# kishwarshafin/pepper

Hardware: AMD Instinct MI355X
Metric: inference windows/sec (whole node) (higher is better)
Workload: dtype f32 via f16 hi/lo split operands (3 MFMAs per product), f32 accumulate

## Files before the change

### pepper_amd/csrc/rnn_h2.hip

```cpp
#include <cstdlib>

#include "common.h"
#include "kernels.h"

namespace {

typedef _Float16 h8 __attribute__((ext_vector_type(8)));
typedef float f32x2 __attribute__((ext_vector_type(2)));

constexpr int MT = 64;

PA_DEV f32x16 mfma_h(h8 a, h8 b, f32x16 c) { return __builtin_amdgcn_mfma_f32_32x32x16_f16(a, b, c, 0, 0, 0); }

PA_DEV void decode_block(int bid, int& dir, int& btile) {
    const int xcd = bid & 7, q = bid >> 3;
    dir = xcd >> 2;
    btile = q * 4 + (xcd & 3);
}


extern __shared__ __attribute__((aligned(16))) uint32_t lds[];
template <int MTILES, int KXROW = 0, int XRD_ = 0>
struct LstmLds {
    static_assert(MTILES == 1 || MTILES == 2, "32 or 64 rows per workgroup");
    static constexpr int H = 256, NW = H / 32;
    static constexpr int MTL = 32 * MTILES;
    static constexpr int ROWB = (H + KXROW) * 4 + 16;
    static constexpr int ROWD = ROWB / 4;
    static_assert((ROWB / 16) % 2 == 1, "row stride must be an odd number of 16-byte slots");
    static constexpr int CS = NW * MTILES * 16 * 64;
    static constexpr int XRD = XRD_, XSLOT = MTL * XRD;
    static constexpr int RING = MTL * ROWD + CS;
    static constexpr size_t BYTES = (size_t)(RING + 2 * XSLOT) * 4;
    static_assert(BYTES <= 160 * 1024, "a workgroup has one CU's 160 KB of LDS");
    PA_DEV static float* c_slots(int u, int lane) { return reinterpret_cast<float*>(lds + MTL * ROWD) + u * (MTILES * 16 * 64) + lane; }
    PA_DEV static void clear(int tid) {
        for (int idx = tid; idx < RING; idx += blockDim.x) lds[idx] = 0u;
    }
};

template <int MTILES> using SeedLds = LstmLds<MTILES>;
template <int MTILES> using EncLds = LstmLds<MTILES, 32>;
template <int MTILES> using DecLds = LstmLds<MTILES, 0, 36>;

PA_DEV f32x2 lstm_gate_pair(f32x2 ai, f32x2 af, f32x2 ag, f32x2 ao, float* c) {
    const f32x2 one = {1.0f, 1.0f};
    auto ex2 = [](f32x2 v) { return f32x2{__builtin_amdgcn_exp2f(v.x), __builtin_amdgcn_exp2f(v.y)}; };
    auto rcp = [](f32x2 v) { return f32x2{__builtin_amdgcn_rcpf(v.x), __builtin_amdgcn_rcpf(v.y)}; };
    const f32x2 ig = rcp(one + ex2(ai));
    const f32x2 fg = rcp(one + ex2(af));
    const f32x2 gg = one - 2.0f * rcp(one + ex2(ag));
    const f32x2 og = rcp(one + ex2(ao));
    const f32x2 cold = {c[0], c[64]};
    const f32x2 cn = fg * cold + ig * gg;
    c[0] = cn.x;
    c[64] = cn.y;
    return og * (one - 2.0f * rcp(one + ex2(cn * 2.8853900817779268f)));
}

template <int ROWD, int MTL, int AUX>
struct YCopy {
    static constexpr int CPR = 256 / 4;
    static constexpr int YROWS = 512 / CPR;
    static constexpr int YC = MTL / YROWS;
    const uint32_t* src;
    __amdgpu_buffer_rsrc_t rs;
    unsigned off;
    int T, ldy;
    PA_DEV YCopy(uint32_t* Y, int ldy_, int b0, int T_, int dir, int tid) : T(T_), ldy(ldy_) {
        const int row = tid / CPR, c = tid % CPR;
        src = lds + row * ROWD + c * 4;
        rs = __builtin_amdgcn_make_buffer_rsrc(Y + (size_t)b0 * T * ldy + dir * 256, 0, 0x7fffffff, 0x00020000);
        off = ((unsigned)(row * T) * ldy + c * 4) * 4u;
    }
    PA_DEV u32x4 read(int j) const { return *reinterpret_cast<const u32x4*>(src + j * YROWS * ROWD); }
    PA_DEV void write(int j, int tp, u32x4 v) const {
        __builtin_amdgcn_raw_buffer_store_b128(v, rs, off, ((unsigned)(j * YROWS * T + tp) * ldy) * 4u, AUX);
    }
};

template <int MTILES>
__global__ __launch_bounds__(512, 1) void lstm_seed_h2_kernel(const float* __restrict__ Xp, int ldx, const uint32_t* __restrict__ Wp,
                                                              uint32_t* __restrict__ Y, int ldy, int B, int T,
                                                              unsigned long long* __restrict__ dbg) {
    using L = SeedLds<MTILES>;
    constexpr int H = 256, KS = H / 16, NT = H / 32;
    constexpr int MTL = L::MTL, ROWD = L::ROWD;
    static_assert(KS % 2 == 0, "the weight prefetch assumes an even number of k steps");

    int dir, btile;
    decode_block(blockIdx.x, dir, btile);
    const int b0 = btile * MTL;
    if (b0 >= B) return;

    const int tid = threadIdx.x, lane = tid & 63;
    const int u = __builtin_amdgcn_readfirstlane(tid >> 6);
    const int li = lane & 31, hf = lane >> 5;
    float* cs = L::c_slots(u, lane);
    L::clear(tid);

    f32x16 acc[MTILES][4];

    const __amdgpu_buffer_rsrc_t xrs = __builtin_amdgcn_make_buffer_rsrc(
        const_cast<float*>(Xp + (size_t)(b0 >> 5) * T * (ldx >> 5) * 1024), 0, 0x7fffffff, 0x00020000);
    const __amdgpu_buffer_rsrc_t wrs = __builtin_amdgcn_make_buffer_rsrc(
        const_cast<uint32_t*>(Wp + ((size_t)dir * (4 * NT) + u) * KS * 512), 0, 0x7fffffff, 0x00020000);
    const unsigned xoff = lane * 16u;
    const unsigned woff = lane * 16u;

    auto seed_chunk = [&](int m, int qd, int t) {
#pragma unroll
        for (int g = 0; g < 4; ++g) {
            const unsigned ct = (unsigned)(dir * (4 * NT) + g * NT + u);
            const unsigned so = (((unsigned)(m * T + t) * (ldx >> 5) + ct) * 4u + qd) * 1024u;
            const f32x4 v = __builtin_bit_cast(f32x4, __builtin_amdgcn_raw_buffer_load_b128(xrs, xoff, so, 0));
            acc[m][g][4 * qd] = v.x;
            acc[m][g][4 * qd + 1] = v.y;
            acc[m][g][4 * qd + 2] = v.z;
            acc[m][g][4 * qd + 3] = v.w;
        }
    };

    struct Frag { h8 b[4][2], a[MTILES][2]; };
    const uint32_t* arow = lds + li * ROWD + hf * 8;
    auto load_b = [&](int s, Frag& fr) {
#pragma unroll
        for (int g = 0; g < 4; ++g)
#pragma unroll
            for (int hl = 0; hl < 2; ++hl)
                fr.b[g][hl] = __builtin_bit_cast(h8, __builtin_amdgcn_raw_buffer_load_b128(
                                                         wrs, woff, (unsigned)((g * NT * KS + s) * 2 + hl) * 1024u, 0));
    };
    auto load_a = [&](int s, Frag& fr) {
#pragma unroll
        for (int m = 0; m < MTILES; ++m) {
            fr.a[m][0] = *reinterpret_cast<const h8*>(arow + m * 32 * ROWD + s * 16);
            fr.a[m][1] = *reinterpret_cast<const h8*>(arow + m * 32 * ROWD + s * 16 + 4);
        }
    };

    const YCopy<ROWD, MTL, 0> yc(Y, ldy, b0, T, dir, tid);
    constexpr int YC = decltype(yc)::YC;

    const int hcol = 32 * u + li;
    unsigned short* hl_dst = reinterpret_cast<unsigned short*>(lds + 4 * hf * ROWD + (hcol >> 3) * 8 + ((hcol & 7) >> 1)) + (hcol & 1);

    Frag ring[2];
    __syncthreads();
    {
        const int t0 = dir ? T - 1 : 0;
#pragma unroll
        for (int m = 0; m < MTILES; ++m)
#pragma unroll
            for (int qd = 0; qd < 4; ++qd) seed_chunk(m, qd, t0);
        load_b(0, ring[0]);
    }
    __syncthreads();

    for (int step = 0; step < T; ++step) {
        const int t = dir ? T - 1 - step : step;
        const bool stamp = dbg != nullptr && blockIdx.x == 8 && lane == 0;
        if (stamp) dbg[(u * 80 + 2 * step) * 2] = __builtin_amdgcn_s_memtime();
        {
            load_a(0, ring[0]);
            const int tp = step > 0 ? (dir ? t + 1 : t - 1) : t;
            u32x4 ycv = {0, 0, 0, 0};
#pragma unroll
            for (int s = 0; s < KS; ++s) {
                const int p = s & 1;
                if (s + 1 < KS) { load_b(s + 1, ring[p ^ 1]); load_a(s + 1, ring[p ^ 1]); }
                else load_b(0, ring[p ^ 1]);
                if (s >= 1 && s <= YC) yc.write(s - 1, tp, ycv);
                if (s < YC) ycv = yc.read(s);
#pragma unroll
                for (int term = 0; term < 3; ++term)
#pragma unroll
                    for (int g = 0; g < 4; ++g)
#pragma unroll
                        for (int m = 0; m < MTILES; ++m)
                            acc[m][g] = mfma_h(ring[p].a[m][term == 0 ? 1 : 0], ring[p].b[g][term == 1 ? 1 : 0], acc[m][g]);
                if (MTILES == 1 && s + 1 < KS) {
#pragma unroll
                    for (int q = 0; q < 8; ++q) {
                        __builtin_amdgcn_sched_group_barrier(0x008, 1, 0);
                        __builtin_amdgcn_sched_group_barrier(0x020, 1, 0);
                    }
#pragma unroll
                    for (int q = 0; q < 2; ++q) {
                        __builtin_amdgcn_sched_group_barrier(0x008, 1, 0);
                        __builtin_amdgcn_sched_group_barrier(0x100, 1, 0);
                    }
                    if (s <= YC) {
                        __builtin_amdgcn_sched_group_barrier(0x008, 1, 0);
                        __builtin_amdgcn_sched_group_barrier(0x040, 1, 0);
                        __builtin_amdgcn_sched_group_barrier(0x008, 1, 0);
                        __builtin_amdgcn_sched_group_barrier(0x100, 1, 0);
                    } else {
                        __builtin_amdgcn_sched_group_barrier(0x008, 2, 0);
                    }
                } else if (s + 1 < KS) {
#pragma unroll
                    for (int q = 0; q < 8; ++q) {
                        __builtin_amdgcn_sched_group_barrier(0x008, 2, 0);
                        __builtin_amdgcn_sched_group_barrier(0x020, 1, 0);
                    }
#pragma unroll
                    for (int q = 0; q < 4; ++q) {
                        __builtin_amdgcn_sched_group_barrier(0x008, 1, 0);
                        __builtin_amdgcn_sched_group_barrier(0x100, 1, 0);
                    }
                    if (s <= YC) {
                        __builtin_amdgcn_sched_group_barrier(0x008, 1, 0);
                        __builtin_amdgcn_sched_group_barrier(0x040, 1, 0);
                        __builtin_amdgcn_sched_group_barrier(0x008, 1, 0);
                        __builtin_amdgcn_sched_group_barrier(0x100, 1, 0);
                        __builtin_amdgcn_sched_group_barrier(0x008, 2, 0);
                    } else {
                        __builtin_amdgcn_sched_group_barrier(0x008, 4, 0);
                    }
                } else if (MTILES == 1) {
#pragma unroll
                    for (int q = 0; q < 8; ++q) {
                        __builtin_amdgcn_sched_group_barrier(0x008, 1, 0);
                        __builtin_amdgcn_sched_group_barrier(0x020, 1, 0);
                    }
                    __builtin_amdgcn_sched_group_barrier(0x008, 4, 0);
                } else {
#pragma unroll
                    for (int q = 0; q < 8; ++q) {
                        __builtin_amdgcn_sched_group_barrier(0x008, 2, 0);
                        __builtin_amdgcn_sched_group_barrier(0x020, 1, 0);
                    }
                    __builtin_amdgcn_sched_group_barrier(0x008, 8, 0);
                }
                __builtin_amdgcn_sched_barrier(0);
            }
        }
        if (stamp) dbg[(u * 80 + 2 * step) * 2 + 1] = __builtin_amdgcn_s_memtime();

        lds_barrier();
        if (stamp) dbg[(u * 80 + 2 * step + 1) * 2] = __builtin_amdgcn_s_memtime();

        const int tn = dir ? t - 1 : t + 1;
#pragma unroll
        for (int m = 0; m < MTILES; ++m)
#pragma unroll
            for (int qd = 0; qd < 4; ++qd) {
#pragma unroll
                for (int e = 0; e < 4; e += 2) {
                    const int r = 4 * qd + e;
                    const f32x2 ai = {acc[m][0][r], acc[m][0][r + 1]}, af = {acc[m][1][r], acc[m][1][r + 1]},
                                ag = {acc[m][2][r], acc[m][2][r + 1]}, ao = {acc[m][3][r], acc[m][3][r + 1]};
                    const f32x2 hv2 = lstm_gate_pair(ai, af, ag, ao, cs + (m * 16 + r) * 64);
#pragma unroll
                    for (int k = 0; k < 2; ++k)
                        h2_store16(hl_dst + (32 * m + ((r + k) & 3) + 8 * ((r + k) >> 2)) * ROWD * 2, k ? hv2.y : hv2.x);
                }
                if (step + 1 < T) seed_chunk(m, qd, tn);
            }
        if (stamp) dbg[(u * 80 + 2 * step + 1) * 2 + 1] = __builtin_amdgcn_s_memtime();
        lds_barrier();
    }
    {
        const int tl = dir ? 0 : T - 1;
#pragma unroll
        for (int j = 0; j < YC; ++j) yc.write(j, tl, yc.read(j));
    }
}


template <int KS>
PA_DEV __amdgpu_buffer_rsrc_t frag16_rsrc(const uint32_t* Wp, int dir, int u) {
    return __builtin_amdgcn_make_buffer_rsrc(const_cast<uint32_t*>(Wp + ((size_t)dir * (4 * 16) + 2 * u) * KS * 512), 0, 0x7fffffff,
                                             0x00020000);
}
template <int KS>
PA_DEV void load_b16(h8 (&b)[2][2][2][2], __amdgpu_buffer_rsrc_t wrs, unsigned woff, int s, int gp, int idx) {
    const int c = idx >> 2, hl = (idx >> 1) & 1, g2 = idx & 1;
    b[gp][g2][c][hl] = __builtin_bit_cast(
        h8, __builtin_amdgcn_raw_buffer_load_b128(wrs, woff, (unsigned)((((2 * gp + g2) * 16 + c) * KS + s) * 2 + hl) * 1024u, 0));
}
PA_DEV __amdgpu_buffer_rsrc_t bias16_rsrc(const float* bias, int dir, int u) {
    return __builtin_amdgcn_make_buffer_rsrc(const_cast<float*>(bias + dir * 4 * 256 + 32 * u), 0, 0x7fffffff, 0x00020000);
}
PA_DEV void load_bias16(float (&cb)[4][2], __amdgpu_buffer_rsrc_t brs, int lr) {
#pragma unroll
    for (int g = 0; g < 4; ++g)
#pragma unroll
        for (int c = 0; c < 2; ++c)
            cb[g][c] = __builtin_bit_cast(float, __builtin_amdgcn_raw_buffer_load_b32(brs, lr * 4u, (unsigned)(g * 256 + 16 * c) * 4u, 0));
}
template <int ROWD>
PA_DEV unsigned short* hl_dst16(int hcol, int lq) {
    return reinterpret_cast<unsigned short*>(lds + 4 * lq * ROWD + (hcol >> 3) * 8 + ((hcol & 7) >> 1)) + (hcol & 1);
}
template <int ROWD, bool ADD_BIAS>
PA_DEV void gate_tile16(f32x4 i4, f32x4 f4, f32x4 g4, f32x4 o4, f32x4 b4, float* cs, unsigned short* dst) {
#pragma unroll
    for (int e = 0; e < 4; e += 2) {
        f32x2 ai = {i4[e], i4[e + 1]}, af = {f4[e], f4[e + 1]}, ag = {g4[e], g4[e + 1]}, ao = {o4[e], o4[e + 1]};
        if (ADD_BIAS) { ai += b4[0]; af += b4[1]; ag += b4[2]; ao += b4[3]; }
        const f32x2 hv2 = lstm_gate_pair(ai, af, ag, ao, cs + e * 64);
#pragma unroll
        for (int k = 0; k < 2; ++k) h2_store16(dst + (e + k) * ROWD * 2, k ? hv2.y : hv2.x);
    }
}

template <bool FRESH_, bool Y_, bool Y2_, int XR_, int AN_>
struct DecStep {
    static constexpr bool FRESH = FRESH_, Y = Y_, Y2 = Y2_;
    static constexpr int XR = XR_, AN = AN_;
};

template <int MTILES>
PA_DEV void lstm_dec_h2_body(const uint32_t* __restrict__ Xh, int ldxh, const float* __restrict__ bias,
                             const uint32_t* __restrict__ Wp, uint32_t* __restrict__ Y, int ldy, int B, int T,
                             unsigned long long* __restrict__ dbg) {
    using L = DecLds<MTILES>;
    constexpr int H = 256, KX = 512, KS = (H + KX) / 32, KSH = H / 32, SAUX = 2;
    constexpr int MTL = L::MTL, RT = 2 * MTILES, ROWD = L::ROWD, XRD = L::XRD, XSLOT = L::XSLOT;

    int dir, btile;
    decode_block(blockIdx.x, dir, btile);
    const int b0 = btile * MTL;
    if (b0 >= B) return;

    const int tid = threadIdx.x, lane = tid & 63;
    const int u = __builtin_amdgcn_readfirstlane(tid >> 6);
    const int lr = lane & 15, lq = lane >> 4;
    float* cs = L::c_slots(u, lane);
    L::clear(tid);
    uint32_t* xring = lds + L::RING;

    f32x4 acc[RT][4][2];

    const __amdgpu_buffer_rsrc_t brs = bias16_rsrc(bias, dir, u);
    const __amdgpu_buffer_rsrc_t wrs = frag16_rsrc<KS>(Wp, dir, u);
    const unsigned woff = lane * 16u;

    const bool xg_stager = tid < MTL * 8;
    const __amdgpu_buffer_rsrc_t xgrs =
        __builtin_amdgcn_make_buffer_rsrc(const_cast<uint32_t*>(Xh + (size_t)b0 * T * ldxh), 0, 0x7fffffff, 0x00020000);
    const unsigned xg_off = ((unsigned)((tid >> 3) * T) * ldxh) * 4u + (tid & 7) * 16u;
    uint32_t* xst_dst = xring + (tid >> 3) * XRD + (tid & 7) * 4;
    u32x4 xstage = {0, 0, 0, 0};
    auto xg_load = [&](int j, int t) {
        if (MTILES == 2 || xg_stager)
            xstage = __builtin_amdgcn_raw_buffer_load_b128(xgrs, xg_off, ((unsigned)t * ldxh) * 4u + (unsigned)j * 128u, SAUX);
    };
    auto xg_store = [&](int slot) {
        if (MTILES == 2 || xg_stager) *reinterpret_cast<u32x4*>(xst_dst + slot * XSLOT) = xstage;
    };

    int once = 1;
    asm volatile("" : "+s"(once));
    h8 a[RT][2];
    h8 b[2][2][2][2];
    const uint32_t* arow = lds + lr * ROWD + lq * 8;
    const uint32_t* xrow = xring + lr * XRD + lq * 8;
    auto load_b = [&](int s, int gp, int idx) { load_b16<KS>(b, wrs, woff, s, gp, idx); };
    auto load_a_h = [&](int s, int m, int hl) { a[m][hl] = *reinterpret_cast<const h8*>(arow + m * 16 * ROWD + s * 32 + hl * 4); };
    auto load_a_x = [&](int slot, int m, int hl) {
        a[m][hl] = *reinterpret_cast<const h8*>(xrow + slot * XSLOT + m * 16 * XRD + hl * 4);
    };

    const YCopy<ROWD, MTL, SAUX> yc(Y, ldy, b0, T, dir, tid);
    constexpr int YC = decltype(yc)::YC;
    unsigned short* hl_dst = hl_dst16<ROWD>(32 * u + lr, lq);

    __syncthreads();
#pragma unroll
    for (int i = 0; i < 8; ++i) load_b(0, 0, i);
    __syncthreads();

    for (int step = 0; step < T; ++step) {
        const int t = dir ? T - 1 - step : step;
        const bool stamp = dbg != nullptr && blockIdx.x == 8 && lane == 0;
        if (stamp) dbg[(u * 80 + 2 * step) * 2] = __builtin_amdgcn_s_memtime();
        {
            const int tp = step > 0 ? (dir ? t + 1 : t - 1) : t;
            u32x4 ycv = {0, 0, 0, 0}, ycv2 = {0, 0, 0, 0};
            constexpr int NM = RT * 12;
            auto kstep = [&](int s, auto cfg) {
                using C = decltype(cfg);
                const int sn = C::AN == 0 ? 0 : s + 1, slot = (s - KSH + 1) & 1;
#pragma unroll
                for (int gp = 0; gp < 2; ++gp) {
                    if (gp == 1 && C::XR == 2) lds_barrier();
#pragma unroll
                    for (int i = 0; i < NM; ++i) {
                        const int m = i / 12, c = (i % 12) / 6, term = (i % 6) >> 1, g2 = i & 1, g = 2 * gp + g2;
                        acc[m][g][c] = __builtin_amdgcn_mfma_f32_16x16x32_f16(a[m][term == 0 ? 1 : 0], b[gp][g2][c][term == 1 ? 1 : 0],
                                                                              C::FRESH && term == 0 ? f32x4{} : acc[m][g][c], 0, 0, 0);
                        if (MTILES == 2 ? (i < 24 && i % 3 == 1) : i < 8) load_b(gp == 0 ? s : sn, gp ^ 1, MTILES == 2 ? i / 3 : i);
                        if (gp == 1 && C::AN != 0 && (i % 12 == 9 || i % 12 == 11)) {
                            if (C::AN == 1) load_a_h(sn, m, i % 12 == 9 ? 1 : 0);
                            else load_a_x(slot, m, i % 12 == 9 ? 1 : 0);
                        }
                        if (C::Y && i == NM / 2 + 1) {
                            if (gp == 0) ycv = yc.read(s);
                            else yc.write(s, tp, ycv);
                        }
                        if (C::Y2 && i == NM / 2 + 4) {
                            if (gp == 0) ycv2 = yc.read(YC - 1);
                            else yc.write(YC - 1, tp, ycv2);
                        }
                        if (C::XR == 2 && gp == 0 && i == NM - 1) xg_store(slot);
                        if (C::XR != 0 && gp == 1 && i == (MTILES == 2 ? 2 : 10)) xg_load(s - 6 < KS - KSH ? s - 6 : KS - KSH - 1, t);
                        __builtin_amdgcn_sched_barrier(0);
                    }
                }
            };
            constexpr bool Y2 = YC > 7;
            constexpr int YL = YC < 6 ? YC : 6;
#pragma unroll
            for (int i = 0; i < 2 * RT; ++i) load_a_h(0, i >> 1, i & 1);
            __builtin_amdgcn_sched_barrier(0);
#pragma unroll 1
            for (int r = 0; r < once; ++r) kstep(0, DecStep<true, true, Y2, 0, 1>{});
#pragma unroll 1
            for (int s = 1; s < YL; ++s) kstep(s, DecStep<false, true, false, 0, 1>{});
#pragma unroll 1
            for (int s = YL; s < 6; ++s) kstep(s, DecStep<false, false, false, 0, 1>{});
#pragma unroll 1
            for (int r = 0; r < once; ++r) kstep(6, DecStep<false, (YC > 6), false, 1, 1>{});
#pragma unroll 1
            for (int s = 7; s < KS - 1; ++s) kstep(s, DecStep<false, false, false, 2, 2>{});
#pragma unroll 1
            for (int r = 0; r < once; ++r) kstep(KS - 1, DecStep<false, false, false, 0, 0>{});
        }
        float cb[4][2];
        load_bias16(cb, brs, lr);
        if (stamp) dbg[(u * 80 + 2 * step) * 2 + 1] = __builtin_amdgcn_s_memtime();

        lds_barrier();
        if (stamp) dbg[(u * 80 + 2 * step + 1) * 2] = __builtin_amdgcn_s_memtime();

#pragma unroll
        for (int m = 0; m < RT; ++m)
#pragma unroll
            for (int c = 0; c < 2; ++c)
                gate_tile16<ROWD, true>(acc[m][0][c], acc[m][1][c], acc[m][2][c], acc[m][3][c], f32x4{cb[0][c], cb[1][c], cb[2][c], cb[3][c]},
                                        cs + (m * 8 + c * 4) * 64, hl_dst + 16 * m * ROWD * 2 + c * 32);
        if (stamp) dbg[(u * 80 + 2 * step + 1) * 2 + 1] = __builtin_amdgcn_s_memtime();
        lds_barrier();
    }
    {
        const int tl = dir ? 0 : T - 1;
#pragma unroll
        for (int j = 0; j < YC; ++j) yc.write(j, tl, yc.read(j));
    }
}

template <bool FRESH_, bool Y_, bool X_, int AN_>
struct EncStep {
    static constexpr bool FRESH = FRESH_, Y = Y_, X = X_;
    static constexpr int AN = AN_;
};

template <int MTILES, bool BC>
PA_DEV void lstm_enc_h2_body(const int8_t* __restrict__ Xi, int F, const float* __restrict__ bias, const uint32_t* __restrict__ Wp,
                             uint32_t* __restrict__ Y, int ldy, int B, int T, unsigned long long* __restrict__ dbg) {
    constexpr int H = 256, KX = 32, KS = (H + KX) / 32, KSH = H / 32, NW = H / 32, SAUX = 2;
    using L = EncLds<MTILES>;
    constexpr int MTL = L::MTL, RT = 2 * MTILES, ROWD = L::ROWD;

    int dir, btile;
    decode_block(blockIdx.x, dir, btile);
    const int b0 = btile * MTL;
    if (b0 >= B) return;

    const int tid = threadIdx.x, lane = tid & 63;
    const int u = __builtin_amdgcn_readfirstlane(tid >> 6);
    const int lr = lane & 15, lq = lane >> 4;
    float* cs = L::c_slots(u, lane);
    L::clear(tid);

    f32x4 acc[RT][4][2];

    const __amdgpu_buffer_rsrc_t brs = bias16_rsrc(bias, dir, u);
    const __amdgpu_buffer_rsrc_t wrs = frag16_rsrc<KS>(Wp, dir, u);
    const unsigned woff = lane * 16u;

    constexpr int XN = (MTL * KX / 2) / (NW * 64);
    unsigned xv[XN];
    auto x_load = [&](int t) {
#pragma unroll
        for (int k = 0; k < XN; ++k) {
            const int e = tid + k * (NW * 64);
            const int row = e / (KX / 2), f = (e % (KX / 2)) * 2;
            int brow = b0 + row;
            brow = brow < B ? brow : B - 1;
            const int8_t* src = Xi + ((size_t)brow * T + t) * F;
            const _Float16 one = BC ? (_Float16)1.0f : (_Float16)0.0f;
            const _Float16 h0 = f < F ? (_Float16)(float)src[f] : (f == F ? one : (_Float16)0.0f);
            const _Float16 h1 = f + 1 < F ? (_Float16)(float)src[f + 1] : (f + 1 == F ? one : (_Float16)0.0f);
            xv[k] = (unsigned)__builtin_bit_cast(unsigned short, h0) | ((unsigned)__builtin_bit_cast(unsigned short, h1) << 16);
        }
    };
    auto x_store = [&]() {
#pragma unroll
        for (int k = 0; k < XN; ++k) {
            const int e = tid + k * (NW * 64);
            const int row = e / (KX / 2), f = (e % (KX / 2)) * 2;
            lds[row * ROWD + ((H + f) >> 3) * 8 + ((f & 7) >> 1)] = xv[k];
        }
    };

    int once = 1;
    asm volatile("" : "+s"(once));
    h8 a[RT][2];
    h8 b[2][2][2][2];
    const uint32_t* arow = lds + lr * ROWD + lq * 8;
    auto load_b = [&](int s, int gp, int idx) { load_b16<KS>(b, wrs, woff, s, gp, idx); };
    auto load_a = [&](int s, int m, int hl) { a[m][hl] = *reinterpret_cast<const h8*>(arow + m * 16 * ROWD + s * 32 + hl * 4); };

    const YCopy<ROWD, MTL, SAUX> yc(Y, ldy, b0, T, dir, tid);
    constexpr int YC = decltype(yc)::YC;
    static_assert(YC <= KSH, "one y copy pass per h k step");
    unsigned short* hl_dst = hl_dst16<ROWD>(32 * u + lr, lq);

    __syncthreads();
    {
        x_load(dir ? T - 1 : 0);
        x_store();
#pragma unroll
        for (int i = 0; i < 8; ++i) load_b(KS - 1, 0, i);
    }
    __syncthreads();

    for (int step = 0; step < T; ++step) {
        const int t = dir ? T - 1 - step : step;
        const bool stamp = dbg != nullptr && blockIdx.x == 8 && lane == 0;
        if (stamp) dbg[(u * 80 + 2 * step) * 2] = __builtin_amdgcn_s_memtime();
        {
            const int tp = step > 0 ? (dir ? t + 1 : t - 1) : t;
            u32x4 ycv = {0, 0, 0, 0};
            auto kstep = [&](int s, auto cfg) {
                using C = decltype(cfg);
                constexpr int PT = C::X ? 4 : 6;
                constexpr int NM = RT * 2 * PT;
                const int sn = C::X ? 0 : s + 1;
#pragma unroll
                for (int gp = 0; gp < 2; ++gp) {
#pragma unroll
                    for (int i = 0; i < NM; ++i) {
                        const int m = i / (2 * PT), c = (i % (2 * PT)) / PT, term = ((i % PT) >> 1) + (C::X ? 1 : 0), g2 = i & 1,
                                  g = 2 * gp + g2;
                        acc[m][g][c] = __builtin_amdgcn_mfma_f32_16x16x32_f16(a[m][term == 0 ? 1 : 0], b[gp][g2][c][term == 1 ? 1 : 0],
                                                                              C::FRESH && i % PT < 2 ? f32x4{} : acc[m][g][c], 0, 0, 0);
                        if (C::X) {
                            if (MTILES == 2 ? (i < 16 && (i & 1)) : i < 8) load_b(gp == 0 ? s : sn, gp ^ 1, MTILES == 2 ? i >> 1 : i);
                        } else {
                            if (MTILES == 2 ? (i < 24 && i % 3 == 1) : i < 8) load_b(gp == 0 ? s : sn, gp ^ 1, MTILES == 2 ? i / 3 : i);
                        }
                        if (!C::X && gp == 1 && C::AN == 1 && i % 12 == 9) load_a(sn, m, 1);
                        if (!C::X && gp == 1 && C::AN != 0 && i % 12 == 11) load_a(sn, m, 0);
                        if (C::Y && i == NM / 2 + 1) {
                            if (gp == 0) ycv = yc.read(s);
                            else yc.write(s, tp, ycv);
                        }
                        __builtin_amdgcn_sched_barrier(0);
                    }
                }
            };
            const int hrun = step == 0 ? 0 : once;
#pragma unroll
            for (int i = 0; i < 2 * RT; ++i) load_a(0, i >> 1, i & 1);
            __builtin_amdgcn_sched_barrier(0);
#pragma unroll 1
            for (int r = 0; r < hrun; ++r) kstep(0, EncStep<true, true, false, 1>{});
#pragma unroll 1
            for (int s = 1; s < (YC < KSH - 1 ? YC : KSH - 1) * hrun; ++s) kstep(s, EncStep<false, true, false, 1>{});
            if constexpr (YC < KSH - 1) {
#pragma unroll 1
                for (int s = YC; s < (KSH - 1) * hrun; ++s) kstep(s, EncStep<false, false, false, 1>{});
            }
#pragma unroll 1
            for (int r = 0; r < hrun; ++r) kstep(KSH - 1, EncStep<false, (YC >= KSH), false, 2>{});
#pragma unroll 1
            for (int r = 0; r < hrun; ++r) kstep(KS - 1, EncStep<false, false, true, 0>{});
#pragma unroll 1
            for (int r = hrun; r < once; ++r) {
#pragma unroll
                for (int m = 0; m < RT; ++m) load_a(KSH, m, 0);
                __builtin_amdgcn_sched_barrier(0);
                kstep(KS - 1, EncStep<true, false, true, 0>{});
            }
        }
        float cb[4][2] = {};
        if (!BC) load_bias16(cb, brs, lr);
        if (stamp) dbg[(u * 80 + 2 * step) * 2 + 1] = __builtin_amdgcn_s_memtime();

        lds_barrier();
        if (stamp) dbg[(u * 80 + 2 * step + 1) * 2] = __builtin_amdgcn_s_memtime();

        const int tn = dir ? t - 1 : t + 1;
        if (step + 1 < T) x_load(tn);
#pragma unroll
        for (int m = 0; m < RT; ++m)
#pragma unroll
            for (int c = 0; c < 2; ++c)
                gate_tile16<ROWD, !BC>(acc[m][0][c], acc[m][1][c], acc[m][2][c], acc[m][3][c], f32x4{cb[0][c], cb[1][c], cb[2][c], cb[3][c]},
                                       cs + (m * 8 + c * 4) * 64, hl_dst + 16 * m * ROWD * 2 + c * 32);
        if (step + 1 < T) x_store();
        if (stamp) dbg[(u * 80 + 2 * step + 1) * 2 + 1] = __builtin_amdgcn_s_memtime();
        lds_barrier();
    }
    {
        const int tl = dir ? 0 : T - 1;
#pragma unroll
        for (int j = 0; j < YC; ++j) yc.write(j, tl, yc.read(j));
    }
}

template <int MTILES>
__global__ __launch_bounds__(512, 1) void lstm_dec_h2_kernel(const uint32_t* __restrict__ Xh, int ldxh, const float* __restrict__ bias,
                                                             const uint32_t* __restrict__ Wp, uint32_t* __restrict__ Y, int ldy,
                                                             int B, int T, unsigned long long* __restrict__ dbg) {
    lstm_dec_h2_body<MTILES>(Xh, ldxh, bias, Wp, Y, ldy, B, T, dbg);
}
template <int MTILES, bool BC>
__global__ __launch_bounds__(512, 1) void lstm_enc_h2_kernel(const int8_t* __restrict__ Xi, int F, const float* __restrict__ bias,
                                                             const uint32_t* __restrict__ Wp, uint32_t* __restrict__ Y, int ldy,
                                                             int B, int T, unsigned long long* __restrict__ dbg) {
    lstm_enc_h2_body<MTILES, BC>(Xi, F, bias, Wp, Y, ldy, B, T, dbg);
}

constexpr int US_AUX_SC1 = 16;

template <int H, int NTW>
__global__ __launch_bounds__(256, 1) void lstm_rec_h2_split_kernel(const float* __restrict__ Xp, int ldx,
                                                                   const uint32_t* __restrict__ Wp, uint32_t* __restrict__ Y,
                                                                   int ldy, int B, int T, uint32_t* __restrict__ exch,
                                                                   unsigned* __restrict__ counters, int* __restrict__ failed,
                                                                   int tiles4, int sabotage) {
    static_assert(H == 256 && (NTW == 1 || NTW == 2), "eight members of 32 units or four of 64");
    constexpr int KS = H / 16, NT = H / 32, K = NT / NTW;
    constexpr int ROWB = H * 4 + 16, ROWD = ROWB / 4;
    extern __shared__ __attribute__((aligned(16))) uint32_t lds[];
    float* gbuf = reinterpret_cast<float*>(lds + 32 * ROWD);
    uint32_t* flag = lds + 32 * ROWD + 4 * NTW * 16 * 64;

    const int xcd = blockIdx.x & 7, q = blockIdx.x >> 3;
    const int dir = xcd >> 2, member = q % K, btile = (q / K) * 4 + (xcd & 3);
    const int b0 = btile * 32;
    if (b0 >= B) return;
    const int group = dir * tiles4 + btile;

    const int tid = threadIdx.x, lane = tid & 63;
    const int w = __builtin_amdgcn_readfirstlane(tid >> 6);
    const int li = lane & 31, hf = lane >> 5;
    for (int idx = tid; idx < 32 * ROWD; idx += 256) lds[idx] = 0u;
    if (tid == 0) *flag = 0u;

    h8 bw[NTW][KS][2];
    {
        const __amdgpu_buffer_rsrc_t wrs = __builtin_amdgcn_make_buffer_rsrc(
            const_cast<uint32_t*>(Wp + (size_t)dir * (4 * NT) * KS * 512), 0, 0x7fffffff, 0x00020000);
#pragma unroll
        for (int j = 0; j < NTW; ++j)
#pragma unroll
            for (int s = 0; s < KS; ++s)
#pragma unroll
                for (int hl = 0; hl < 2; ++hl)
                    bw[j][s][hl] = __builtin_bit_cast(h8, __builtin_amdgcn_raw_buffer_load_b128(
                                                              wrs, lane * 16u,
                                                              (unsigned)(((w * NT + member * NTW + j) * KS + s) * 2 + hl) * 1024u, 0));
    }
    const __amdgpu_buffer_rsrc_t xrs = __builtin_amdgcn_make_buffer_rsrc(
        const_cast<float*>(Xp + (size_t)btile * T * (ldx >> 5) * 1024), 0, 0x7fffffff, 0x00020000);
    const unsigned ct0 = (unsigned)(dir * (4 * NT) + w * NT + member * NTW);
    f32x16 acc[NTW];
    auto seed = [&](int t) {
#pragma unroll
        for (int j = 0; j < NTW; ++j)
#pragma unroll
            for (int qd = 0; qd < 4; ++qd) {
                const unsigned so = (((unsigned)t * (ldx >> 5) + ct0 + j) * 4u + qd) * 1024u;
                const f32x4 v = __builtin_bit_cast(f32x4, __builtin_amdgcn_raw_buffer_load_b128(xrs, lane * 16u, so, 0));
                acc[j][4 * qd] = v.x;
                acc[j][4 * qd + 1] = v.y;
                acc[j][4 * qd + 2] = v.z;
                acc[j][4 * qd + 3] = v.w;
            }
    };

    const uint32_t* arow = lds + li * ROWD + hf * 8;
    const int hcol = 32 * member * NTW + li;
    unsigned short* hl_dst = reinterpret_cast<unsigned short*>(lds + 4 * hf * ROWD + (hcol >> 3) * 8 + ((hcol & 7) >> 1)) + (hcol & 1);
    const int xrow = tid >> 3, xc = tid & 7;
    const __amdgpu_buffer_rsrc_t ers = __builtin_amdgcn_make_buffer_rsrc(
        exch + (size_t)group * 2 * 32 * H, 0, 0x7fffffff, 0x00020000);
    const __amdgpu_buffer_rsrc_t yrs = __builtin_amdgcn_make_buffer_rsrc(
        Y + (size_t)b0 * T * ldy + dir * H, 0, 0x7fffffff, 0x00020000);
    unsigned* cnt = counters + group * 32;

    float c[NTW][4];
#pragma unroll
    for (int j = 0; j < NTW; ++j)
#pragma unroll
        for (int e = 0; e < 4; ++e) c[j][e] = 0.0f;
    seed(dir ? T - 1 : 0);
    __syncthreads();

    for (int step = 0; step < T; ++step) {
        const int t = dir ? T - 1 - step : step;
        {
            h8 a0 = *reinterpret_cast<const h8*>(arow), a1 = *reinterpret_cast<const h8*>(arow + 4);
#pragma unroll
            for (int s = 0; s < KS; ++s) {
                h8 n0 = a0, n1 = a1;
                if (s + 1 < KS) {
                    n0 = *reinterpret_cast<const h8*>(arow + (s + 1) * 16);
                    n1 = *reinterpret_cast<const h8*>(arow + (s + 1) * 16 + 4);
                }
#pragma unroll
                for (int j = 0; j < NTW; ++j) acc[j] = mfma_h(a1, bw[j][s][0], acc[j]);
#pragma unroll
                for (int j = 0; j < NTW; ++j) acc[j] = mfma_h(a0, bw[j][s][1], acc[j]);
#pragma unroll
                for (int j = 0; j < NTW; ++j) acc[j] = mfma_h(a0, bw[j][s][0], acc[j]);
                a0 = n0;
                a1 = n1;
            }
        }
#pragma unroll
        for (int j = 0; j < NTW; ++j)
#pragma unroll
            for (int r = 0; r < 16; ++r) {
// ... 892 lines not shown
```

Measured before the change: 2.796 million.

## Skip zero-state recurrent MFMAs at first decoder step and triple-buffer x slots

At the first decoder timestep the hidden state is zero, so the h-part k-steps are skipped and accumulation starts fresh from the x-input k-steps, with the initial B prefetch moved to the first x k-step. The x staging ring grows from two to three LDS slots, and the global load and LDS store of x fragments are issued earlier in the k-step. This removes redundant MFMA work on step zero and gives x loads more time in flight, at the cost of extra LDS and a more complex step-zero path that must correctly seed the ring.

After: 2.814 million (median of 6 runs). Within noise of the previous version (+0.6%).

```diff
diff --git a/pepper_amd/csrc/rnn_h2.hip b/pepper_amd/csrc/rnn_h2.hip
--- a/pepper_amd/csrc/rnn_h2.hip
+++ b/pepper_amd/csrc/rnn_h2.hip
@@ -20,7 +20,7 @@
 
 
 extern __shared__ __attribute__((aligned(16))) uint32_t lds[];
-template <int MTILES, int KXROW = 0, int XRD_ = 0>
+template <int MTILES, int KXROW = 0, int XRD_ = 0, int XSLOTS_ = 2>
 struct LstmLds {
     static_assert(MTILES == 1 || MTILES == 2, "32 or 64 rows per workgroup");
     static constexpr int H = 256, NW = H / 32;
@@ -31,7 +31,8 @@
     static constexpr int CS = NW * MTILES * 16 * 64;
     static constexpr int XRD = XRD_, XSLOT = MTL * XRD;
     static constexpr int RING = MTL * ROWD + CS;
-    static constexpr size_t BYTES = (size_t)(RING + 2 * XSLOT) * 4;
+    static constexpr int XSLOTS = XSLOTS_;
+    static constexpr size_t BYTES = (size_t)(RING + XSLOTS * XSLOT) * 4;
     static_assert(BYTES <= 160 * 1024, "a workgroup has one CU's 160 KB of LDS");
     PA_DEV static float* c_slots(int u, int lane) { return reinterpret_cast<float*>(lds + MTL * ROWD) + u * (MTILES * 16 * 64) + lane; }
     PA_DEV static void clear(int tid) {
@@ -41,7 +42,7 @@
 
 template <int MTILES> using SeedLds = LstmLds<MTILES>;
 template <int MTILES> using EncLds = LstmLds<MTILES, 32>;
-template <int MTILES> using DecLds = LstmLds<MTILES, 0, 36>;
+template <int MTILES> using DecLds = LstmLds<MTILES, 0, 36, 3>;
 
 PA_DEV f32x2 lstm_gate_pair(f32x2 ai, f32x2 af, f32x2 ag, f32x2 ao, float* c) {
     const f32x2 one = {1.0f, 1.0f};
@@ -306,6 +307,9 @@
     }
 }
 
+#ifndef PA_DEC_SKIP0
+#define PA_DEC_SKIP0 1
+#endif
 template <bool FRESH_, bool Y_, bool Y2_, int XR_, int AN_>
 struct DecStep {
     static constexpr bool FRESH = FRESH_, Y = Y_, Y2 = Y2_;
@@ -319,6 +323,8 @@
     using L = DecLds<MTILES>;
     constexpr int H = 256, KX = 512, KS = (H + KX) / 32, KSH = H / 32, SAUX = 2;
     constexpr int MTL = L::MTL, RT = 2 * MTILES, ROWD = L::ROWD, XRD = L::XRD, XSLOT = L::XSLOT;
+    constexpr int XSLOTS = L::XSLOTS;
+    constexpr bool SKIP0 = PA_DEC_SKIP0 != 0;
 
     int dir, btile;
     decode_block(blockIdx.x, dir, btile);
@@ -370,7 +376,7 @@
 
     __syncthreads();
 #pragma unroll
-    for (int i = 0; i < 8; ++i) load_b(0, 0, i);
+    for (int i = 0; i < 8; ++i) load_b(SKIP0 ? KSH : 0, 0, i);
     __syncthreads();
 
     for (int step = 0; step < T; ++step) {
@@ -381,9 +387,11 @@
             const int tp = step > 0 ? (dir ? t + 1 : t - 1) : t;
             u32x4 ycv = {0, 0, 0, 0}, ycv2 = {0, 0, 0, 0};
             constexpr int NM = RT * 12;
+            constexpr int XW = MTILES == 2 ? 0 : 8, XL = XW + 2;
             auto kstep = [&](int s, auto cfg) {
                 using C = decltype(cfg);
-                const int sn = C::AN == 0 ? 0 : s + 1, slot = (s - KSH + 1) & 1;
+                const int sn = C::AN == 0 ? 0 : s + 1;
+                const int slot = C::XR == 2 ? (s - KSH + 1) % XSLOTS : 0;
 #pragma unroll
                 for (int gp = 0; gp < 2; ++gp) {
                     if (gp == 1 && C::XR == 2) lds_barrier();
@@ -405,8 +413,8 @@
                             if (gp == 0) ycv2 = yc.read(YC - 1);
                             else yc.write(YC - 1, tp, ycv2);
                         }
-                        if (C::XR == 2 && gp == 0 && i == NM - 1) xg_store(slot);
-                        if (C::XR != 0 && gp == 1 && i == (MTILES == 2 ? 2 : 10)) xg_load(s - 6 < KS - KSH ? s - 6 : KS - KSH - 1, t);
+                        if (C::XR == 2 && gp == 0 && i == XW) xg_store(slot);
+                        if (C::XR != 0 && gp == 0 && i == XL) xg_load(s - 6 < KS - KSH ? s - 6 : KS - KSH - 1, t);
                         __builtin_amdgcn_sched_barrier(0);
                     }
                 }
@@ -416,16 +424,32 @@
 #pragma unroll
             for (int i = 0; i < 2 * RT; ++i) load_a_h(0, i >> 1, i & 1);
             __builtin_amdgcn_sched_barrier(0);
+            const int hrun = SKIP0 && step == 0 ? 0 : once;
 #pragma unroll 1
-            for (int r = 0; r < once; ++r) kstep(0, DecStep<true, true, Y2, 0, 1>{});
+            for (int r = 0; r < hrun; ++r) kstep(0, DecStep<true, true, Y2, 0, 1>{});
 #pragma unroll 1
-            for (int s = 1; s < YL; ++s) kstep(s, DecStep<false, true, false, 0, 1>{});
+            for (int s = 1; s < YL * hrun; ++s) kstep(s, DecStep<false, true, false, 0, 1>{});
+            if constexpr (YL < 6) {
 #pragma unroll 1
-            for (int s = YL; s < 6; ++s) kstep(s, DecStep<false, false, false, 0, 1>{});
+                for (int s = YL; s < 6 * hrun; ++s) kstep(s, DecStep<false, false, false, 0, 1>{});
+            }
 #pragma unroll 1
-            for (int r = 0; r < once; ++r) kstep(6, DecStep<false, (YC > 6), false, 1, 1>{});
+            for (int r = 0; r < hrun; ++r) kstep(6, DecStep<false, (YC > 6), false, 1, 1>{});
+            if constexpr (SKIP0) {
 #pragma unroll 1
-            for (int s = 7; s < KS - 1; ++s) kstep(s, DecStep<false, false, false, 2, 2>{});
+                for (int r = hrun; r < once; ++r) {
+                    xg_load(0, t);
+                    xg_store(0);
+                    xg_load(1, t);
+                    lds_barrier();
+#pragma unroll
+                    for (int i = 0; i < 2 * RT; ++i) load_a_x(0, i >> 1, i & 1);
+                    __builtin_amdgcn_sched_barrier(0);
+                    kstep(KSH, DecStep<true, false, false, 2, 2>{});
+                }
+            }
+#pragma unroll 1
+            for (int s = KSH + 1 - 2 * hrun; s < KS - 1; ++s) kstep(s, DecStep<false, false, false, 2, 2>{});
 #pragma unroll 1
             for (int r = 0; r < once; ++r) kstep(KS - 1, DecStep<false, false, false, 0, 0>{});
         }
```
